# choyingw/SynergyNet

Measured on AMD Instinct MI355X. Metric: faces/sec (120x120, 68-lmk + 53215-vert), higher is better.
Workload: dtype f32 (fp16x2 split operands, fp32 accumulate)

## Files before the change

### synergynet_amd/csrc/fused_block_lb4.hip

```cpp
#include "syn_internal.h"

#include <cstdio>
#include <cstdlib>
#include <type_traits>

namespace syn {

typedef float f32x4 __attribute__((ext_vector_type(4)));
typedef float f32x2 __attribute__((ext_vector_type(2)));
typedef unsigned u32x4 __attribute__((ext_vector_type(4)));
typedef unsigned u32x2 __attribute__((ext_vector_type(2)));
typedef _Float16 f16x8 __attribute__((ext_vector_type(8)));
typedef _Float16 f16x2 __attribute__((ext_vector_type(2)));

namespace {
__device__ __forceinline__ void split2q(float x0, float x1, unsigned &a, unsigned &b) {
    a = __builtin_bit_cast(unsigned, __builtin_amdgcn_cvt_pkrtz(x0, x1));
    float r0, r1;
    asm("v_fma_mix_f32 %0, %1, -1.0, %2 op_sel_hi:[1,0,0]" : "=v"(r0) : "v"(a), "v"(x0));
    asm("v_fma_mix_f32 %0, %1, -1.0, %2 op_sel:[1,0,0] op_sel_hi:[1,0,0]" : "=v"(r1) : "v"(a), "v"(x1));
    b = __builtin_bit_cast(unsigned, __builtin_amdgcn_cvt_pkrtz(r0, r1));
}
__device__ __forceinline__ void split2w(float x0, float x1, u32x4 (&pc)[2], int d) {
    unsigned a, b;
    split2q(x0, x1, a, b);
    pc[0][d] = a; pc[1][d] = b;
}
__device__ __forceinline__ f32x4 mfmaq(u32x4 a, u32x4 b, f32x4 c) {
    return __builtin_amdgcn_mfma_f32_16x16x32_f16(__builtin_bit_cast(f16x8, a), __builtin_bit_cast(f16x8, b), c, 0, 0, 0);
}
template <int CTRL>
__device__ __forceinline__ float dppq(float x) {
    return __builtin_bit_cast(float, __builtin_amdgcn_mov_dpp(__builtin_bit_cast(int, x), CTRL, 0xf, 0xf, true));
}
template <int CTRL>
__device__ __forceinline__ f32x2 dppq2(f32x2 v) {
    f32x2 r;
    r[0] = dppq<CTRL>(v[0]);
    r[1] = dppq<CTRL>(v[1]);
    return r;
}
constexpr int kShr1 = 0x111, kShl1 = 0x101, kShr4 = 0x114, kShl4 = 0x104;
}

template <int CIN_, int HID_, int COUT_, bool RES_>
struct Lb4Cfg {
    static constexpr int CIN = CIN_, HID = HID_, COUT = COUT_;
    static constexpr bool RES = RES_;
    static constexpr int KE = CIN / 32, NG = HID / 32, MT = COUT / 16, MTW = MT / 2;
    static constexpr int WE_DW = 2 * KE * 2 * 256, WP_DW = MT * 2 * 256, TB_DW = 2 * 256;
    static constexpr int NKB = ((WE_DW + WP_DW + TB_DW) / 256 + 7) / 8 * 8;
    static constexpr int GRP_DW = NKB * 256;
    static constexpr int XCH_DW = 4 * 2 * 64 * 4;
    static constexpr int LDS_DW = 2 * GRP_DW + XCH_DW;
    static_assert(CIN % 32 == 0 && HID % 32 == 0 && COUT % 32 == 0, "k32 steps, groups, two halves of the output tiles");
    static_assert(!RES || CIN == COUT, "residual only on same-width blocks");
    static_assert(LDS_DW * 4 <= 160 * 1024, "LDS budget");
};

struct Lb4NoNext { static constexpr int NKB = 0; };
struct Lb4StageArgs {
    const float *X;
    const unsigned *Glb;
    const float *p_shift;
    float *Y;
    float *part = nullptr;
    int g0 = 0, g1 = 0;
};

template <int N>
__device__ __forceinline__ void lb4_fetch(u32x4 *pf, const unsigned *src , int wave) {
#pragma unroll
    for (int i = 0; i < N; ++i) pf[i] = *(const u32x4 *)(src + (wave + 8 * i) * 256);
}
template <int N>
__device__ __forceinline__ void lb4_park(const u32x4 *pf, unsigned *dst , int wave) {
#pragma unroll
    for (int i = 0; i < N; ++i) *(u32x4 *)&dst[(wave + 8 * i) * 256] = pf[i];
}

template <class C, class CN, bool FIRST, int GRPL, bool PARTIAL = false>
__device__ __forceinline__ void lb4_stage(unsigned *smem, const Lb4StageArgs &sa, const unsigned *GlbNext, int B, u32x4 (&Xr)[5][2], f32x4 (&vres)[5]) {
    constexpr int KE = C::KE, MTW = C::MTW, CIN = C::CIN, COUT = C::COUT;
    constexpr bool HANDOFF = !__is_same(CN, void);
    static_assert(KE == 5 && C::NG % 2 == 0, "160 input channels; the double buffer's parity carries over to the next stage");
    const float *__restrict__ X = sa.X, *__restrict__ p_shift = sa.p_shift;
    const unsigned *__restrict__ Glb = sa.Glb;
    float *__restrict__ Y = sa.Y;
    const int tid = threadIdx.x, lane = tid & 63;
    const int wave = __builtin_amdgcn_readfirstlane(tid >> 6);
    const int fl = wave >> 1, t = wave & 1;
    const int f = blockIdx.x * 4 + fl;
    const bool real = f < B;
    const int fc = real ? f : B - 1;
    const int n = lane & 15, g = lane >> 4;
    const unsigned l4 = lane * 4, g4 = g * 4;
    unsigned *Xch = smem + 2 * GRPL;

    constexpr int NPW = C::NKB / 8;
    using CNX = typename std::conditional<HANDOFF, CN, Lb4NoNext>::type;
    constexpr int NPWN = CNX::NKB / 8;
    u32x4 pf[NPW > NPWN ? NPW : NPWN];
    const int gsl = PARTIAL ? (sa.g1 - sa.g0) : C::NG;
    const int gb = PARTIAL ? (int)blockIdx.y * gsl : 0, ge = gb + gsl;
    if (FIRST) {
        lb4_fetch<NPW>(pf, Glb + (size_t)gb * C::GRP_DW + l4, wave);
        f32x4 xv[KE][2];
#pragma unroll
        for (int kc = 0; kc < KE; ++kc) {
            const float *src = X + ((size_t)fc * 16 + n) * CIN + 32 * kc + 8 * g;
            xv[kc][0] = *(const f32x4 *)src;
            xv[kc][1] = *(const f32x4 *)(src + 4);
        }
#pragma unroll
        for (int kc = 0; kc < KE; ++kc) {
            f32x4 a = xv[kc][0] * 16.0f, b = xv[kc][1] * 16.0f;
            if (!real) { a = (f32x4){0.f, 0.f, 0.f, 0.f}; b = a; }
            split2w(a[0], a[1], Xr[kc], 0);
            split2w(a[2], a[3], Xr[kc], 1);
            split2w(b[0], b[1], Xr[kc], 2);
            split2w(b[2], b[3], Xr[kc], 3);
        }
    }
    const float mL = (n & 3) != 0 ? 1.f : 0.f, mR = (n & 3) != 3 ? 1.f : 0.f;
    f32x4 acc[MTW];
#pragma unroll
    for (int i = 0; i < MTW; ++i) acc[i] = (f32x4){0.f, 0.f, 0.f, 0.f};
    float c6e = 0.f, inv_p = 0.f;
    if (FIRST) lb4_park<NPW>(pf, smem + l4, wave);

    {
        const float *t0 = reinterpret_cast<const float *>(Glb + C::WE_DW + C::WP_DW);
        c6e = t0[11 * 32]; inv_p = t0[11 * 32 + 1];
    }
    for (int G = gb; G < ge; ++G) {
        __syncthreads();
        if (G + 1 < ge) lb4_fetch<NPW>(pf, Glb + (size_t)(G + 1) * C::GRP_DW + l4, wave);
        else if (HANDOFF) lb4_fetch<NPWN>(pf, GlbNext + l4, wave);
        const unsigned *We = smem + ((G - gb) & 1) * GRPL, *Wp = We + C::WE_DW;
        const float *Tb = reinterpret_cast<const float *>(Wp + C::WP_DW);
        __builtin_amdgcn_sched_barrier(0);
        u32x4 Ae[KE][2], Ap[MTW][2];
        f32x4 D = *(const f32x4 *)&Tb[10 * 32 + 16 * t + g4];
#pragma unroll
        for (int kc = 0; kc < KE; ++kc)
#pragma unroll
            for (int p = 1; p >= 0; --p) Ae[kc][p] = *(const u32x4 *)&We[((t * KE + kc) * 2 + p) * 256 + l4];
        constexpr int MTW0 = MTW > 5 ? MTW / 2 : MTW;
        f32x2 wt[2][9], dsht[2];
#pragma unroll
        for (int hf = 0; hf < 2; ++hf) {
#pragma unroll
            for (int k = 0; k < 9; ++k) wt[hf][k] = *(const f32x2 *)&Tb[k * 32 + 16 * t + 2 * hf + g4];
            dsht[hf] = *(const f32x2 *)&Tb[9 * 32 + 16 * t + 2 * hf + g4];
        }
        __builtin_amdgcn_sched_barrier(0);
#pragma unroll
        for (int kc = 0; kc < KE; ++kc) {
            D = mfmaq(Ae[kc][1], Xr[kc][0], D);
            D = mfmaq(Ae[kc][0], Xr[kc][1], D);
            D = mfmaq(Ae[kc][0], Xr[kc][0], D);
        }
        __builtin_amdgcn_sched_barrier(0);
#pragma unroll
        for (int i = 0; i < MTW0; ++i)
#pragma unroll
            for (int p = 0; p < 2; ++p) Ap[i][p] = *(const u32x4 *)&Wp[((t * MTW + i) * 2 + p) * 256 + l4];
        __builtin_amdgcn_sched_barrier(0);
        u32x4 own;
#pragma unroll
        for (int hf = 0; hf < 2; ++hf) {
            const f32x2 (&w)[9] = wt[hf];
            const f32x2 dsh = dsht[hf];
            f32x2 E;
            E[0] = __builtin_amdgcn_fmed3f(D[2 * hf] * c6e, 0.0f, 1.0f);
            E[1] = __builtin_amdgcn_fmed3f(D[2 * hf + 1] * c6e, 0.0f, 1.0f);
            const f32x2 l = dppq2<kShr1>(E) * mL, rt = dppq2<kShl1>(E) * mR;
            f32x2 H[3];
#pragma unroll
            for (int dy = 0; dy < 3; ++dy) {
                H[dy] = l * w[3 * dy];
                H[dy] += E * w[3 * dy + 1];
                H[dy] += rt * w[3 * dy + 2];
            }
            f32x2 O = dsh + dppq2<kShr4>(H[0]);
            O += H[1];
            {
                const f32x2 h2 = dppq2<kShl4>(H[2]);
                asm("v_pk_add_f32 %0, %1, %2 clamp" : "=v"(O) : "v"(O), "v"(h2));
            }
            unsigned a, b;
            split2q(O[0], O[1], a, b);
            own[hf] = a; own[2 + hf] = b;
        }
        *(u32x4 *)&Xch[((fl * 2 + t) * 64 + lane) * 4] = own;
        __syncthreads();
        const u32x4 oth = *(const u32x4 *)&Xch[((fl * 2 + (1 - t)) * 64 + lane) * 4];
#pragma unroll
        for (int i = MTW0; i < MTW; ++i)
#pragma unroll
            for (int p = 0; p < 2; ++p) Ap[i][p] = *(const u32x4 *)&Wp[((t * MTW + i) * 2 + p) * 256 + l4];
        u32x4 Bd[2];
        Bd[0] = t == 0 ? (u32x4){own[0], own[1], oth[0], oth[1]} : (u32x4){oth[0], oth[1], own[0], own[1]};
        Bd[1] = t == 0 ? (u32x4){own[2], own[3], oth[2], oth[3]} : (u32x4){oth[2], oth[3], own[2], own[3]};
#pragma unroll
        for (int i = 0; i < MTW; ++i) {
            acc[i] = mfmaq(Ap[i][1], Bd[0], acc[i]);
            acc[i] = mfmaq(Ap[i][0], Bd[1], acc[i]);
            acc[i] = mfmaq(Ap[i][0], Bd[0], acc[i]);
        }
        if (G + 1 < ge) lb4_park<NPW>(pf, smem + ((G + 1 - gb) & 1) * GRPL + l4, wave);
        else if (HANDOFF) lb4_park<NPWN>(pf, smem + l4, wave);
    }
    if constexpr (PARTIAL) {
        if (real) {
#pragma unroll
            for (int i = 0; i < MTW; ++i)
                *(f32x4 *)&sa.part[(((size_t)blockIdx.y * B + f) * 16 + n) * COUT + 16 * (t * MTW + i) + g4] = acc[i];
        }
        return;
    }

    f32x4 vout[MTW];
#pragma unroll
    for (int i = 0; i < MTW; ++i) {
        const int nch = 16 * (t * MTW + i) + g4;
        const size_t at = ((size_t)fc * 16 + n) * COUT + nch;
        f32x4 v = acc[i] * inv_p + *(const f32x4 *)&p_shift[nch];
        if constexpr (C::RES) {
            if (FIRST) v += *(const f32x4 *)&X[at];
            else v += vres[i];
        }
        if (!HANDOFF && real) *(f32x4 *)&Y[at] = v;
        vout[i] = v;
    }
    if constexpr (HANDOFF) {
        static_assert(CN::CIN == COUT && MTW == 5, "the next block takes this block's output: five output tiles per wave");
        unsigned *HO = smem + GRPL;
        __syncthreads();
#pragma unroll
        for (int i = 0; i < MTW; ++i) {
            vres[i] = vout[i];
            const int mt = t * MTW + i, kc = mt >> 1, lt = (2 * (mt & 1) + (g >> 1)) * 16 + n, dw = 2 * (g & 1);
            const f32x4 v = real ? vout[i] * 16.0f : (f32x4){0.f, 0.f, 0.f, 0.f};
            unsigned a0, b0, a1, b1;
            split2q(v[0], v[1], a0, b0);
            split2q(v[2], v[3], a1, b1);
            *(u32x2 *)&HO[((fl * KE + kc) * 2 + 0) * 256 + lt * 4 + dw] = (u32x2){a0, a1};
            *(u32x2 *)&HO[((fl * KE + kc) * 2 + 1) * 256 + lt * 4 + dw] = (u32x2){b0, b1};
        }
        __syncthreads();
#pragma unroll
        for (int kc = 0; kc < KE; ++kc)
#pragma unroll
            for (int p = 0; p < 2; ++p) Xr[kc][p] = *(const u32x4 *)&HO[((fl * KE + kc) * 2 + p) * 256 + l4];
    }
}

template <class C, bool PARTIAL = false>
__global__ __launch_bounds__(512) __attribute__((amdgpu_waves_per_eu(2, 2)))
void fused_block_lb4_kernel(Lb4StageArgs sa, int B) {
    __shared__ __attribute__((aligned(16))) unsigned smem[C::LDS_DW];
    u32x4 Xr[5][2];
    f32x4 vres[5];
    lb4_stage<C, void, true, C::GRP_DW, PARTIAL>(smem, sa, nullptr, B, Xr, vres);
}

template <class C>
__global__ __launch_bounds__(256) void lb4_reduce_kernel(const float *__restrict__ part, int S, const unsigned *__restrict__ Glb,
                                                         const float *__restrict__ p_shift, const float *__restrict__ X,
                                                         float *__restrict__ Y, int B) {
    constexpr int C4 = C::COUT / 4;
    const long idx = (long)blockIdx.x * 256 + threadIdx.x, total = (long)B * 16 * C4;
    if (idx >= total) return;
    const int c4 = (int)(idx % C4);
    const float inv_p = reinterpret_cast<const float *>(Glb + C::WE_DW + C::WP_DW)[11 * 32 + 1];
    f32x4 a = *(const f32x4 *)&part[(size_t)idx * 4];
    for (int sl = 1; sl < S; ++sl) a += *(const f32x4 *)&part[((size_t)sl * total + idx) * 4];
    f32x4 v = a * inv_p + *(const f32x4 *)&p_shift[4 * c4];
    if (C::RES) v += *(const f32x4 *)&X[(size_t)idx * 4];
    *(f32x4 *)&Y[(size_t)idx * 4] = v;
}

using Q15 = Lb4Cfg<160, 960, 160, true>;
using Q17 = Lb4Cfg<160, 960, 320, false>;

constexpr int kChain4Grp = Q17::GRP_DW > Q15::GRP_DW ? Q17::GRP_DW : Q15::GRP_DW;
constexpr int kChain4LdsDw = 2 * kChain4Grp + Q15::XCH_DW;
static_assert(kChain4LdsDw * 4 <= 160 * 1024 && 4 * 5 * 2 * 256 <= kChain4Grp, "LDS budget; the handed-over fragments of four faces fit one buffer half");
struct Lb4ChainArgs { Lb4StageArgs s[3]; };

__global__ __launch_bounds__(512) __attribute__((amdgpu_waves_per_eu(2, 2)))
void fused_chain_lb4_kernel(Lb4ChainArgs ca, int B) {
    __shared__ __attribute__((aligned(16))) unsigned smem[kChain4LdsDw];
    u32x4 Xr[5][2];
    f32x4 vres[5];
    lb4_stage<Q15, Q15, true, kChain4Grp>(smem, ca.s[0], ca.s[1].Glb, B, Xr, vres);
    lb4_stage<Q15, Q17, false, kChain4Grp>(smem, ca.s[1], ca.s[2].Glb, B, Xr, vres);
    lb4_stage<Q17, void, false, kChain4Grp>(smem, ca.s[2], nullptr, B, Xr, vres);
}

template <class C>
static void launch_lb4(const FusedBlockArgs &a, int B, hipStream_t s) {
    fused_block_lb4_kernel<C><<<(B + 3) / 4, 512, 0, s>>>(Lb4StageArgs{a.X, a.Glb, a.p_shift, a.Y}, B);
}

template <class C>
static bool launch_lb4_sliced(const FusedBlockArgs &a, int B, hipStream_t s) {
    if (!a.scratch) return false;
    const int wg = (B + 3) / 4;
    static const int divs[] = {2, 3, 5, 6, 10, 15, 30};
    int S = 30;
    for (int d : divs) if (wg * d >= 192) { S = d; break; }
    if ((size_t)S * B * 16 * C::COUT > a.scratch_floats) return false;
    Lb4StageArgs sa{a.X, a.Glb, a.p_shift, a.Y};
    sa.part = a.scratch; sa.g0 = 0; sa.g1 = C::NG / S;
    fused_block_lb4_kernel<C, true><<<dim3(wg, S), 512, 0, s>>>(sa, B);
    const long total = (long)B * 16 * (C::COUT / 4);
    lb4_reduce_kernel<C><<<(int)((total + 255) / 256), 256, 0, s>>>(a.scratch, S, a.Glb, a.p_shift, a.X, a.Y, B);
    return true;
}

bool launch_lb4_sliced17_deferred(const FusedBlockArgs &a, int B, hipStream_t s, HeadSliced *out) {
    static const bool on = test_knob("head_sliced_in", 1) != 0;
    static const int wide_min = (int)test_knob("head_wide_min", 513);
    if (!on || !out || !a.Glb || a.prof || !a.scratch || B >= wide_min || B >= 576) return false;
    using C = Q17;
    const int wg = (B + 3) / 4;
    static const int divs[] = {2, 3, 5, 6, 10, 15, 30};
    int S = 30;
    for (int d : divs) if (wg * d >= 192) { S = d; break; }
    if (S > 3) return false;
    if ((size_t)S * B * 16 * C::COUT > a.scratch_floats) return false;
    Lb4StageArgs sa{a.X, a.Glb, a.p_shift, a.Y};
    sa.part = a.scratch; sa.g0 = 0; sa.g1 = C::NG / S;
    fused_block_lb4_kernel<C, true><<<dim3(wg, S), 512, 0, s>>>(sa, B);
    *out = HeadSliced{a.scratch, S, reinterpret_cast<const float *>(a.Glb + C::WE_DW + C::WP_DW) + 11 * 32 + 1, a.p_shift};
    return true;
}

static int lb4_min_batch() {
    constexpr int min_b = 576;
    return min_b;
}

bool launch_fused_chain_lb4(const FusedBlockArgs *a, int B, hipStream_t s) {
    static const int chain = (int)test_knob("lb4_chain", 1);
    if (!chain || B < lb4_min_batch()) return false;
    Lb4ChainArgs ca;
    for (int i = 0; i < 3; ++i) {
        if (!a[i].Glb || a[i].prof) return false;
        ca.s[i] = Lb4StageArgs{a[i].X, a[i].Glb, a[i].p_shift, a[i].Y};
    }
    fused_chain_lb4_kernel<<<(B + 3) / 4, 512, 0, s>>>(ca, B);
    return true;
}

bool launch_fused_block_lb4(int feature, const FusedBlockArgs &a, int B, hipStream_t s) {
    if (!a.Glb || a.prof) return false;
    if (B < lb4_min_batch()) {
        switch (feature) {
            case 15: case 16: return launch_lb4_sliced<Q15>(a, B, s);
            case 17: return launch_lb4_sliced<Q17>(a, B, s);
            default: return false;
        }
    }
    switch (feature) {
        case 15: case 16: launch_lb4<Q15>(a, B, s); return true;
        case 17: launch_lb4<Q17>(a, B, s); return true;
        default: return false;
    }
}

}
```

Baseline: 1.006 million.

## Deepen weight prefetch to two groups and preload next group's fragments during project MFMAs

Restructures the per-group loop of the fused inverted-residual kernel into a software pipeline. Global weight fetches now run two groups ahead via a carried prefetch register array. The next group's expand fragments and depthwise taps are read from LDS interleaved with the current group's project MFMAs, and the project-weight LDS loads are interleaved with the expand MFMAs. Fetch addresses are made wave-uniform with readfirstlane so they go into scalar registers. The aim is to hide LDS and global latency behind MFMA work, at the cost of more live registers, a more complex tail (last two groups are peeled), and extra state (pf, pre) passed across chained stages.

```diff
diff --git a/synergynet_amd/csrc/fused_block_lb4.hip b/synergynet_amd/csrc/fused_block_lb4.hip
--- a/synergynet_amd/csrc/fused_block_lb4.hip
+++ b/synergynet_amd/csrc/fused_block_lb4.hip
@@ -69,9 +69,12 @@
 };
 
 template <int N>
-__device__ __forceinline__ void lb4_fetch(u32x4 *pf, const unsigned *src , int wave) {
-#pragma unroll
-    for (int i = 0; i < N; ++i) pf[i] = *(const u32x4 *)(src + (wave + 8 * i) * 256);
+__device__ __forceinline__ void lb4_fetch(u32x4 *pf, const unsigned *src , unsigned lane16, int wave) {
+    const unsigned long long a = reinterpret_cast<unsigned long long>(src + wave * 256);
+    const unsigned lo = __builtin_amdgcn_readfirstlane((unsigned)a), hi = __builtin_amdgcn_readfirstlane((unsigned)(a >> 32));
+    const char *base = reinterpret_cast<const char *>(((unsigned long long)hi << 32) | lo);
+#pragma unroll
+    for (int i = 0; i < N; ++i) pf[i] = *(const u32x4 *)(base + i * 8192 + lane16);
 }
 template <int N>
 __device__ __forceinline__ void lb4_park(const u32x4 *pf, unsigned *dst , int wave) {
@@ -79,8 +82,31 @@
     for (int i = 0; i < N; ++i) *(u32x4 *)&dst[(wave + 8 * i) * 256] = pf[i];
 }
 
-template <class C, class CN, bool FIRST, int GRPL, bool PARTIAL = false>
-__device__ __forceinline__ void lb4_stage(unsigned *smem, const Lb4StageArgs &sa, const unsigned *GlbNext, int B, u32x4 (&Xr)[5][2], f32x4 (&vres)[5]) {
+struct Lb4Pre {
+    f32x4 D;
+    u32x4 Ae[5][2];
+    f32x4 wr[10];
+};
+constexpr int kLb4PreUnits = 10;
+template <class C>
+__device__ __forceinline__ void lb4_pre_unit(Lb4Pre &pre, const unsigned *half, int u, int t, unsigned l4, unsigned g4) {
+    if (u < 5) {
+        const float *Tb = reinterpret_cast<const float *>(half + C::WE_DW + C::WP_DW);
+        if (u == 0) pre.D = *(const f32x4 *)&Tb[10 * 32 + 16 * t + g4];
+#pragma unroll
+        for (int p = 1; p >= 0; --p) pre.Ae[u][p] = *(const u32x4 *)&half[((t * 5 + u) * 2 + p) * 256 + l4];
+    } else {
+        const float *Tb = reinterpret_cast<const float *>(half + C::WE_DW + C::WP_DW);
+#pragma unroll
+        for (int k = 2 * (u - 5); k < 2 * (u - 5) + 2; ++k) pre.wr[k] = *(const f32x4 *)&Tb[k * 32 + 16 * t + g4];
+    }
+}
+template <class T> struct Lb4Tag { using type = T; };
+template <int N> struct Lb4Int { static constexpr int value = N; };
+
+template <class C, class CN, bool FIRST, int GRPL, bool PARTIAL, int NPF, int PRE0, int LAG>
+__device__ __forceinline__ void lb4_stage(unsigned *smem, const Lb4StageArgs &sa, const unsigned *GlbNext, int B, u32x4 (&Xr)[5][2], f32x4 (&vres)[5],
+                                          u32x4 (&pf)[NPF], Lb4Pre &pre) {
     constexpr int KE = C::KE, MTW = C::MTW, CIN = C::CIN, COUT = C::COUT;
     constexpr bool HANDOFF = !__is_same(CN, void);
     static_assert(KE == 5 && C::NG % 2 == 0, "160 input channels; the double buffer's parity carries over to the next stage");
@@ -94,17 +120,17 @@
     const bool real = f < B;
     const int fc = real ? f : B - 1;
     const int n = lane & 15, g = lane >> 4;
-    const unsigned l4 = lane * 4, g4 = g * 4;
+    const unsigned l4 = lane * 4, g4 = g * 4, l16 = lane * 16;
     unsigned *Xch = smem + 2 * GRPL;
 
     constexpr int NPW = C::NKB / 8;
     using CNX = typename std::conditional<HANDOFF, CN, Lb4NoNext>::type;
     constexpr int NPWN = CNX::NKB / 8;
-    u32x4 pf[NPW > NPWN ? NPW : NPWN];
+    static_assert(NPF >= NPW && NPF >= NPWN, "pf holds a group of this stage or of the next");
     const int gsl = PARTIAL ? (sa.g1 - sa.g0) : C::NG;
     const int gb = PARTIAL ? (int)blockIdx.y * gsl : 0, ge = gb + gsl;
     if (FIRST) {
-        lb4_fetch<NPW>(pf, Glb + (size_t)gb * C::GRP_DW + l4, wave);
+        lb4_fetch<NPW>(pf, Glb + (size_t)gb * C::GRP_DW, l16, wave);
         f32x4 xv[KE][2];
 #pragma unroll
         for (int kc = 0; kc < KE; ++kc) {
@@ -127,51 +153,50 @@
 #pragma unroll
     for (int i = 0; i < MTW; ++i) acc[i] = (f32x4){0.f, 0.f, 0.f, 0.f};
     float c6e = 0.f, inv_p = 0.f;
-    if (FIRST) lb4_park<NPW>(pf, smem + l4, wave);
+    if (FIRST) {
+        lb4_park<NPW>(pf, smem + l4, wave);
+        if (!PARTIAL || gsl >= 2) lb4_fetch<NPW>(pf, Glb + (size_t)(gb + 1) * C::GRP_DW, l16, wave);
+        __syncthreads();
+#pragma unroll
+        for (int u = 0; u < kLb4PreUnits; ++u) lb4_pre_unit<C>(pre, smem, u, t, l4, g4);
+    }
 
     {
         const float *t0 = reinterpret_cast<const float *>(Glb + C::WE_DW + C::WP_DW);
         c6e = t0[11 * 32]; inv_p = t0[11 * 32 + 1];
     }
-    for (int G = gb; G < ge; ++G) {
+    auto group = [&](auto nf_, auto np_, auto cp_, int G, const unsigned *fsrc) __attribute__((always_inline)) {
+        constexpr int NF = decltype(nf_)::value, NP = decltype(np_)::value;
+        using CP = typename decltype(cp_)::type;
+        constexpr bool HASNEXT = !__is_same(CP, void);
         __syncthreads();
-        if (G + 1 < ge) lb4_fetch<NPW>(pf, Glb + (size_t)(G + 1) * C::GRP_DW + l4, wave);
-        else if (HANDOFF) lb4_fetch<NPWN>(pf, GlbNext + l4, wave);
         const unsigned *We = smem + ((G - gb) & 1) * GRPL, *Wp = We + C::WE_DW;
-        const float *Tb = reinterpret_cast<const float *>(Wp + C::WP_DW);
+        unsigned *Wn = smem + ((G + 1 - gb) & 1) * GRPL;
+        u32x4 Ap[MTW][2];
+        f32x4 D = pre.D;
+        constexpr int MTW0 = MTW > 5 ? MTW / 2 : MTW;
+        static_assert(MTW0 == KE, "one output tile's project fragments per k32 step of the expand chain");
+#pragma unroll
+        for (int kc = 0; kc < KE; ++kc) {
+            D = mfmaq(pre.Ae[kc][1], Xr[kc][0], D);
+            D = mfmaq(pre.Ae[kc][0], Xr[kc][1], D);
+            D = mfmaq(pre.Ae[kc][0], Xr[kc][0], D);
+            __builtin_amdgcn_sched_barrier(0);
+#pragma unroll
+            for (int p = 0; p < 2; ++p) Ap[kc][p] = *(const u32x4 *)&Wp[((t * MTW + kc) * 2 + p) * 256 + l4];
+            __builtin_amdgcn_sched_barrier(0);
+        }
+        if (NP) lb4_park<NP>(pf, Wn + l4, wave);
         __builtin_amdgcn_sched_barrier(0);
-        u32x4 Ae[KE][2], Ap[MTW][2];
-        f32x4 D = *(const f32x4 *)&Tb[10 * 32 + 16 * t + g4];
-#pragma unroll
-        for (int kc = 0; kc < KE; ++kc)
-#pragma unroll
-            for (int p = 1; p >= 0; --p) Ae[kc][p] = *(const u32x4 *)&We[((t * KE + kc) * 2 + p) * 256 + l4];
-        constexpr int MTW0 = MTW > 5 ? MTW / 2 : MTW;
-        f32x2 wt[2][9], dsht[2];
-#pragma unroll
-        for (int hf = 0; hf < 2; ++hf) {
-#pragma unroll
-            for (int k = 0; k < 9; ++k) wt[hf][k] = *(const f32x2 *)&Tb[k * 32 + 16 * t + 2 * hf + g4];
-            dsht[hf] = *(const f32x2 *)&Tb[9 * 32 + 16 * t + 2 * hf + g4];
-        }
-        __builtin_amdgcn_sched_barrier(0);
-#pragma unroll
-        for (int kc = 0; kc < KE; ++kc) {
-            D = mfmaq(Ae[kc][1], Xr[kc][0], D);
-            D = mfmaq(Ae[kc][0], Xr[kc][1], D);
-            D = mfmaq(Ae[kc][0], Xr[kc][0], D);
-        }
-        __builtin_amdgcn_sched_barrier(0);
-#pragma unroll
-        for (int i = 0; i < MTW0; ++i)
-#pragma unroll
-            for (int p = 0; p < 2; ++p) Ap[i][p] = *(const u32x4 *)&Wp[((t * MTW + i) * 2 + p) * 256 + l4];
+        if (NF) lb4_fetch<NF>(pf, fsrc, l16, wave);
         __builtin_amdgcn_sched_barrier(0);
         u32x4 own;
 #pragma unroll
         for (int hf = 0; hf < 2; ++hf) {
-            const f32x2 (&w)[9] = wt[hf];
-            const f32x2 dsh = dsht[hf];
+            f32x2 w[9];
+#pragma unroll
+            for (int k = 0; k < 9; ++k) w[k] = (f32x2){pre.wr[k][2 * hf], pre.wr[k][2 * hf + 1]};
+            const f32x2 dsh = (f32x2){pre.wr[9][2 * hf], pre.wr[9][2 * hf + 1]};
             f32x2 E;
             E[0] = __builtin_amdgcn_fmed3f(D[2 * hf] * c6e, 0.0f, 1.0f);
             E[1] = __builtin_amdgcn_fmed3f(D[2 * hf + 1] * c6e, 0.0f, 1.0f);
@@ -204,14 +229,26 @@
         Bd[0] = t == 0 ? (u32x4){own[0], own[1], oth[0], oth[1]} : (u32x4){oth[0], oth[1], own[0], own[1]};
         Bd[1] = t == 0 ? (u32x4){own[2], own[3], oth[2], oth[3]} : (u32x4){oth[2], oth[3], own[2], own[3]};
 #pragma unroll
-        for (int i = 0; i < MTW; ++i) {
+        for (int i = 0; i <= MTW; ++i) {
+            if constexpr (HASNEXT) {
+#pragma unroll
+                for (int u = 0; u < kLb4PreUnits; ++u) {
+                    const int at = u < PRE0 ? 0 : (u - PRE0 + LAG < MTW ? u - PRE0 + LAG : MTW);
+                    if (at == i) lb4_pre_unit<CP>(pre, Wn, u, t, l4, g4);
+                }
+                __builtin_amdgcn_sched_barrier(0);
+            }
+            if (i == MTW) break;
             acc[i] = mfmaq(Ap[i][1], Bd[0], acc[i]);
             acc[i] = mfmaq(Ap[i][0], Bd[1], acc[i]);
             acc[i] = mfmaq(Ap[i][0], Bd[0], acc[i]);
-        }
-        if (G + 1 < ge) lb4_park<NPW>(pf, smem + ((G + 1 - gb) & 1) * GRPL + l4, wave);
-        else if (HANDOFF) lb4_park<NPWN>(pf, smem + l4, wave);
-    }
+            if constexpr (HASNEXT) __builtin_amdgcn_sched_barrier(0);
+        }
+    };
+    for (int G = gb; G < ge - 2; ++G)
+        group(Lb4Int<NPW>{}, Lb4Int<NPW>{}, Lb4Tag<C>{}, G, Glb + (size_t)(G + 2) * C::GRP_DW);
+    if (!PARTIAL || gsl >= 2) group(Lb4Int<NPWN>{}, Lb4Int<NPW>{}, Lb4Tag<C>{}, ge - 2, GlbNext);
+    group(Lb4Int<NPWN>{}, Lb4Int<NPWN>{}, Lb4Tag<CN>{}, ge - 1, HANDOFF ? GlbNext + CNX::NKB * 256 : nullptr);
     if constexpr (PARTIAL) {
         if (real) {
 #pragma unroll
@@ -257,13 +294,16 @@
     }
 }
 
+constexpr int kPre0Q15 = 10, kPre0Q15C = 4, kPre0Q17 = 0, kLagQ15 = 1, kLagQ15C = 1, kLagQ17 = 2;
+
 template <class C, bool PARTIAL = false>
 __global__ __launch_bounds__(512) __attribute__((amdgpu_waves_per_eu(2, 2)))
 void fused_block_lb4_kernel(Lb4StageArgs sa, int B) {
     __shared__ __attribute__((aligned(16))) unsigned smem[C::LDS_DW];
-    u32x4 Xr[5][2];
+    u32x4 Xr[5][2], pf[C::NKB / 8];
     f32x4 vres[5];
-    lb4_stage<C, void, true, C::GRP_DW, PARTIAL>(smem, sa, nullptr, B, Xr, vres);
+    Lb4Pre pre;
+    lb4_stage<C, void, true, C::GRP_DW, PARTIAL, C::NKB / 8, C::MTW == 5 ? kPre0Q15 : kPre0Q17, C::MTW == 5 ? kLagQ15 : kLagQ17>(smem, sa, nullptr, B, Xr, vres, pf, pre);
 }
 
 template <class C>
@@ -293,11 +333,14 @@
 __global__ __launch_bounds__(512) __attribute__((amdgpu_waves_per_eu(2, 2)))
 void fused_chain_lb4_kernel(Lb4ChainArgs ca, int B) {
     __shared__ __attribute__((aligned(16))) unsigned smem[kChain4LdsDw];
-    u32x4 Xr[5][2];
+    constexpr int NPF = Q17::NKB / 8;
+    static_assert(Q17::NKB >= Q15::NKB, "pf holds a group of any stage");
+    u32x4 Xr[5][2], pf[NPF];
     f32x4 vres[5];
-    lb4_stage<Q15, Q15, true, kChain4Grp>(smem, ca.s[0], ca.s[1].Glb, B, Xr, vres);
-    lb4_stage<Q15, Q17, false, kChain4Grp>(smem, ca.s[1], ca.s[2].Glb, B, Xr, vres);
-    lb4_stage<Q17, void, false, kChain4Grp>(smem, ca.s[2], nullptr, B, Xr, vres);
+    Lb4Pre pre;
+    lb4_stage<Q15, Q15, true, kChain4Grp, false, NPF, kPre0Q15C, kLagQ15C>(smem, ca.s[0], ca.s[1].Glb, B, Xr, vres, pf, pre);
+    lb4_stage<Q15, Q17, false, kChain4Grp, false, NPF, kPre0Q15C, kLagQ15C>(smem, ca.s[1], ca.s[2].Glb, B, Xr, vres, pf, pre);
+    lb4_stage<Q17, void, false, kChain4Grp, false, NPF, kPre0Q17, kLagQ17>(smem, ca.s[2], nullptr, B, Xr, vres, pf, pre);
 }
 
 template <class C>
```

Measured after the change: 1.020 million, median of 6. +1.3%, better.
